# HazyResearch/flash-fft-conv

Measured on AMD Instinct MI355X. Metric: FFT-conv fwd+bwd seq/s, B=16 H=768 L=16384 fft=32768 bf16, higher is better.
Workload: dtype bf16; 1 GPU; FlashFFTConv(32768) B=16 H=768 L=16384 bf16, fwd+bwd incl. k->k_f and dk (BASELINE configs[1]); heads_per_rank=768, parallelism=head-shard x1 (no collective)

## Files before the change

flash-fft-conv_amd/csrc/ffc_body.h:

```cpp
#pragma once
#include <stdint.h>

#include "ffc_layout.h"
#include "ffc_plan.h"

#ifndef FFC_FN
#define FFC_FN inline __attribute__((always_inline))
#endif

namespace ffc {

struct ConvArgs {
  const void* u;
  const void* pregate;
  const void* postgate;
  void* y;
  const void* kf;
  const uint8_t* tab;
  PlanTabs t;
  int B, H, L;
  int npair;
  int nchunk, ppc;
  int conj_kf;
  int fast;
// ... 562 lines not shown
    else rows_load<NC>(a, h, pq, un, X);
  }
  template <int NC, bool PL>
  static FFC_FN void rows_store_sel(const ConvArgs& a, int h, int pq, Unit un, const RowRegsT<NC>& X) {
    if constexpr (PL) rows_store_pl<NC>(a, pq, un, X);
    else rows_store<NC>(a, h, pq, un, X);
  }
  template <int NC, bool PL>
  static FFC_FN void rows_in_sel(const ConvArgs& a, int h, int pq, Unit un) {
    RowRegsT<NC> X;
    rows_load_sel<NC, PL>(a, h, pq, un, X);
    rows_store_sel<NC, PL>(a, h, pq, un, X);
  }
  static constexpr bool HAS_DMA = GEO::OUTER && GEO::N1 == 32 && GEO::S1 == 1;
  static constexpr int DMA_ROW0 = GEO::N1 / 2;
  static FFC_FN void rows_dma(const ConvArgs& a, int h, int pq, Unit un) {
    if (a.stream) rows_dma_t<true>(a, h, pq, un);
    else rows_dma_t<false>(a, h, pq, un);
  }
  template <bool NT>
  static FFC_FN void rows_dma_t(const ConvArgs& a, int h, int pq, Unit un) {
    const i32 lane = B::opaque(B::lane());
#pragma unroll
    for (int pl = 0; pl < 2; pl++) {
      const int b = 2 * pq + pl;
      const uint16_t* base = (const uint16_t*)a.u + row_off(b < a.B ? b : a.B - 1, true, a.sbu, h, a.L);
#pragma unroll
      for (int r = 0; r < GEO::N1 / 2; r++) {
        i32 n = B::imin(lane * 2 + (r * GEO::Mi + un.wq * 128), a.L - 2);
        B::template g2lds32<NT>(base, n >> 1, un.eb + pl * GEO::PLANE + (DMA_ROW0 + r) * (GEO::Mi * 2) + un.wq * 256);
      }
    }
  }
  static FFC_FN void rows_dma_finish(const ConvArgs& a, int pq, Unit un) {
    B::vm_wait0();
    const i32 lane = B::opaque(B::lane());
#pragma unroll
    for (int pl = 0; pl < 2; pl++) {
      const bool ok = (2 * pq + pl) < a.B;
#pragma unroll
      for (int r = 0; r < GEO::N1 / 2; r++) {
        if (ok && (r + 1) * GEO::Mi <= a.L) continue;
        i32 n = lane * 2 + (r * GEO::Mi + un.wq * 128);
        B::lds_w32p(lane * 4 + (un.eb + pl * GEO::PLANE + (DMA_ROW0 + r) * (GEO::Mi * 2) + un.wq * 256), B::uconst(0),
                    B::pnot((n < a.L) && ok));
      }
    }
    B::lds_fence();
  }

  static FFC_FN U4 gload8_rows(const uint16_t* base, i32 b, int h, const ConvArgs& a, int64_t sb, i32 n, int fast, pred ok) {
    const int sbi = (int)sb;
    if (fast) {
      i32 o16 = b * (sbi >> 3) + (h * (a.L >> 3) + (n >> 3));
      return B::g_r128p(base, o16, ok && (n < a.L));
    }
    u32 w[4];
#pragma unroll
    for (int q = 0; q < 4; q++) {
      i32 e0 = b * sbi + (h * a.L + n + 2 * q);
      u32 lo = B::g_r16(base, e0, ok && ((n + 2 * q) < a.L));
      u32 hi = B::g_r16(base, e0 + 1, ok && ((n + (2 * q + 1)) < a.L));
      w[q] = lo | (hi << 16);
    }
    U4 v; v.x = w[0]; v.y = w[1]; v.z = w[2]; v.w = w[3];
    return v;
  }
  static FFC_FN void gstore8_rows(uint16_t* base, i32 b, int h, const ConvArgs& a, int64_t sb, i32 n, int fast, pred ok, U4 v) {
// ... 597 lines not shown
            i32 m = j * 4 + (s1 * 128 + w * 128 * GEO::S1 + 2 * tp + th);
            i32 k0 = hi * 4 + ((16 * half) % GEO::N1);
            F2 tr[4], ti[4];
            if constexpr (RP) chain8p(m * (k0 * ps.R + ps.k0), m * ps.R, -1.0f, s_fwd, tr, ti, GEO::N * ps.R - 1, 1.0f / (float)(GEO::N * ps.R));
            else chain8p(m * k0, m, -1.0f, s_fwd, tr, ti);
            apply8(re, im, half, tr, ti);
          }
        }
        if (th == 0) {
          re0 = re; im0 = im;
        } else {
#pragma unroll
          for (int r = 0; r < 16; r++) {
            if (!FWD && HALF && row_dead((r & 3) + 8 * (r >> 2))) continue;
            const u32 vr = B::template pack<DT>(re0[r], re[r]), vi = B::template pack<DT>(im0[r], im[r]);
            if (tp == 0) {
              p0r[r] = vr; p0i[r] = vi;
            } else {
              const int c = (r & 3) + 8 * (r >> 2);
              const int s1 = c / GEO::N1, rwc = c % GEO::N1;
              i32 off = colb[s1] + rwc * (GEO::Mi * 2);
              U2 wr, wi;
              wr.x = p0r[r]; wr.y = vr; wi.x = p0i[r]; wi.y = vi;
              B::lds_w64(off, wr);
              B::lds_w64(off + GEO::PLANE, wi);
            }
          }
        }
      }
    }
  }

  static constexpr bool HALF_C = GEO::N1 == 32 && GEO::N2 == 32 && GEO::N3 == 32;
  using A4 = typename B::A4;
  struct NoMid { FFC_FN void operator()() const {} };
  template <bool GS, class MID>
  static FFC_FN void outer_inv_half_cols(int hc, Unit un, const W4& Cr, const W4& Ci, const W4& Cn, const ConvArgs* a, int h, int pq, MID mid) {
    const i32 lane = B::opaque(B::lane());
    const i32 c = lane & 15, g = lane >> 4;
    const i32 m0 = c * 4 + (hc * 64 + un.wq * 128);
    const i32 colr = e_off<GEO, i32>((g >> 1) * 16 + (g & 1) * 4, m0) + un.eb;
    U2 rawr[8], rawi[8];
#pragma unroll
    for (int e = 0; e < 8; e++) {
      i32 off = colr + kslot_row(0, 0, e) * (GEO::Mi * 2);
      rawr[e] = B::lds_r64(off); rawi[e] = B::lds_r64(off + GEO::PLANE);
    }
    A4 re[4], im[4];
#pragma unroll
    for (int t = 0; t < 4; t++) {
      W4 dr, di;
#pragma unroll
      for (int d = 0; d < 4; d++) {
        const u32 ar = (t & 2) ? rawr[2 * d].y : rawr[2 * d].x, br = (t & 2) ? rawr[2 * d + 1].y : rawr[2 * d + 1].x;
        const u32 ai = (t & 2) ? rawi[2 * d].y : rawi[2 * d].x, bi = (t & 2) ? rawi[2 * d + 1].y : rawi[2 * d + 1].x;
        dr[d] = (t & 1) ? B::merge_hi(ar, br) : B::merge_lo(ar, br);
        di[d] = (t & 1) ? B::merge_hi(ai, bi) : B::merge_lo(ai, bi);
      }
      re[t] = B::a4_zero(); im[t] = B::a4_zero();
      B::template mfma16<DT>(re[t], Cr, dr);
      B::template mfma16<DT>(im[t], Ci, dr);
      B::template mfma16<DT>(re[t], Cn, di);
      B::template mfma16<DT>(im[t], Cr, di);
      if (t == 0) mid();
    }
    U2 wr[4], wi[4];
#pragma unroll
    for (int r = 0; r < 4; r++) {
      wr[r].x = B::template pack<DT>(re[0][r], re[1][r]); wr[r].y = B::template pack<DT>(re[2][r], re[3][r]);
      wi[r].x = B::template pack<DT>(im[0][r], im[1][r]); wi[r].y = B::template pack<DT>(im[2][r], im[3][r]);
    }
    if constexpr (!GS) {
      const i32 colw = e_off<GEO, i32>(g * 4, m0) + un.eb;
#pragma unroll
      for (int r = 0; r < 4; r++) {
        B::lds_w64(colw + r * (GEO::Mi * 2), wr[r]);
        B::lds_w64(colw + (r * (GEO::Mi * 2) + GEO::PLANE), wi[r]);
      }
    } else {
      const i32 n = g * (4 * GEO::Mi) + m0;
#pragma unroll
      for (int pl = 0; pl < 2; pl++) {
        const int b = 2 * pq + pl;
        const bool ok = b < a->B;
        uint16_t* base = (uint16_t*)a->y + row_off(b, ok, a->sby, h, a->L);
        if (a->stream) {
#pragma unroll
          for (int r = 0; r < 4; r++) B::g_w64_nt(base, (n + r * GEO::Mi) >> 2, pl ? wi[r] : wr[r], ((n + r * GEO::Mi) < a->L) && ok);
        } else {
#pragma unroll
          for (int r = 0; r < 4; r++) B::g_w64(base, (n + r * GEO::Mi) >> 2, pl ? wi[r] : wr[r], ((n + r * GEO::Mi) < a->L) && ok);
        }
      }
    }
  }
  template <bool GS>
  static FFC_FN void outer_inv_half(Unit un, const ConvArgs* a = nullptr, int h = 0, int pq = 0) { outer_inv_half<GS>(un, a, h, pq, NoMid()); }
  template <bool GS, class LAST>
  static FFC_FN void outer_inv_half(Unit un, const ConvArgs* a, int h, int pq, LAST last) {
    static_assert(HALF_C && GEO::S1 == 1 && GEO::NW == 8, "half-height phase C: fft 32768");
    static_assert(!GS || !B::HAS_ADD, "the direct store has no addend");
    const i32 lane = B::opaque(B::lane());
    const i32 toff = ((lane & 15) + ((lane >> 4) & 1) * 32) * 16 + (lane >> 5) * 3072 + GEO::L_F1;
    U4 v0 = B::lds_r128(toff), v1 = B::lds_r128(toff + 1024), v2 = B::lds_r128(toff + 2048);
    W4 Cr = B::w4(v0.x, v0.y, v0.z, v0.w);
    W4 Ci = B::w4(v2.x, v2.y, v2.z, v2.w);
    W4 Cn = B::w4(v1.x, v1.y, v1.z, v1.w);
    B::pin(Cr); B::pin(Ci); B::pin(Cn);
    if constexpr (B::LEAN_OUTER) {
#pragma unroll 1
      for (int hc = 0; hc < 2; hc++)
        outer_inv_half_cols<GS>(hc, un, Cr, Ci, Cn, a, h, pq, [&]() { if (hc == 1) last(); });
    } else {
      outer_inv_half_cols<GS>(0, un, Cr, Ci, Cn, a, h, pq, NoMid());
      outer_inv_half_cols<GS>(1, un, Cr, Ci, Cn, a, h, pq, last);
    }
  }

  template <bool FWD, bool HALF, bool RP = false, bool DIN = false, bool NOTW = false>
  static FFC_FN void outer_stage(int L, Unit un, float s_fwd = 1.0f, Pass ps = Pass(), int flags = 0) {
    if constexpr (DIN) { outer_stage_pair<FWD, HALF, RP, true, NOTW>(L, un, s_fwd, ps); return; }
    if constexpr (!FWD && HALF && !RP && HALF_C) {
      if (!(flags & 256)) { outer_inv_half<false>(un); return; }
    }
    if constexpr (B::LEAN_OUTER && !(FWD && HALF && GEO::N1 == 32)) outer_stage_tile<FWD, HALF, RP, NOTW>(L, un, s_fwd, ps);
    else if constexpr (!B::LEAN_OUTER && FFC_OUTER_QUAD != 0 && HALF) outer_stage_quad<FWD, HALF, RP, NOTW>(L, un, s_fwd, ps);
    else outer_stage_pair<FWD, HALF, RP, false, NOTW>(L, un, s_fwd, ps);
  }

  struct InnerRegs { Mat F2; CT16 tw; i32 roff[2][2]; i32 woff[4]; };
  template <bool TWR = true>
  static FFC_FN void load_inner(InnerRegs& R, Unit un) {
    lds_mat(R.F2, GEO::L_F2);
    if constexpr (TWR) lds_ct16(R.tw, GEO::L_TW);
    const i32 lane = B::lane();
    const i32 c = lane & 31, hi = lane >> 5;
    const i32 i16 = lane & 15, g16 = (lane >> 4) & 1;
    const i32 n3b = (g16 * 16) % GEO::N3;
#pragma unroll
    for (int ms = 0; ms < 2; ms++)
#pragma unroll
      for (int rho = 0; rho < 2; rho++) {
        i32 U = hi * 4 + (16 * ms + 8 * rho) + (i16 >> 2);
        i32 sU = U / GEO::N2, n2 = U % GEO::N2;
        i32 row = sU * GEO::SV + ((g16 * 16) / GEO::N3);
        R.roff[ms][rho] = e_off<GEO, i32>(row, n2 * GEO::N3 + n3b + (i16 & 3) * 4) + un.eb;
      }
#pragma unroll
// ... 684 lines not shown
        for (int i = 0; i < 4; i++) B::cmulp(tr[i], ti[i], c16, s16, tr[i], ti[i]);
        apply8(reA, imA, 1, tr, ti);
        apply8(reB, imB, 1, tr, ti);
      } else
#pragma unroll
      for (int half = 0; half < 2; half++) {
        const int sV = (16 * half) / GEO::N3;
        i32 k1 = sUl * GEO::SV + (sV + tau * GEO::G);
        i32 n30 = hi * 4 + ((16 * half) % GEO::N3);
        F2 tr[4], ti[4];
        chain8p(B::mul24(mlane + n30, k1), k1, 1.0f, a.s_inv, tr, ti);
        apply8(reA, imA, half, tr, ti);
        apply8(reB, imB, half, tr, ti);
      }
    }
    tile_store(tau, R, reA, imA);
    tile_store(tau, R, reB, imB, DB);
  }

  static FFC_FN void unit_barrier() {
    if constexpr (GEO::NW > 1) B::barrier();
    else B::lds_fence();
  }
  template <bool HALF, bool PROF = false, bool RP = false, bool SZ = false, bool SP = false, bool GS = false, bool PL = false>
  static FFC_FN void outer_jobs(const ConvArgs& a, int h, int p0, int p1, int u, Unit un, int wg_linear = 0) {
    static_assert(!GS || (HALF && !RP && !SP && HALF_C), "direct-store phase C: single-pass fft 32768, L <= N/2");
    static_assert(!PL || GS, "plain input rows: a form of the direct-store kernels");
    constexpr int NC = HALF ? NCH / 2 : NCH;
    constexpr bool PREFETCH = HALF && !RP;
    constexpr bool FOLDF = CAN_FOLD && !RP && !SP && !PROF && !B::LEAN_OUTER;
    constexpr bool CROSS = !SP && !RP && !PROF && !B::LEAN_OUTER && GEO::N3 == GEO::N2 && GEO::NW > 1 && GEO::UPW >= 2;
    const int npass = RP ? a.R : 1;
    const int iters = ((p1 - p0 + GEO::UPW - 1) / GEO::UPW) * npass;
    RowRegsT<NC> X;
    if constexpr (PREFETCH) { if (p0 + u < p1) rows_load_sel<NC, PL>(a, h, p0 + u, un, X); }
    unsigned long long acc[8] = {0, 0, 0, 0, 0, 0, 0, 0}, t0 = 0, t1 = 0;
#define FFC_TICK(k) if (PROF) { t1 = B::clock(); acc[k] += t1 - t0; t0 = t1; }
    const bool second = B::wave() >= 4;
#define FFC_PRIO(x) if constexpr (GEO::NW > 1) B::template setprio<x>();
#pragma unroll 1
    for (int it = 0; it < iters; it++) {
      const int p = p0 + (RP ? it / npass : it) * GEO::UPW + u;
      const Pass ps = RP ? make_pass(a, it % npass) : Pass();
      const int hk = RP ? h * ps.R + ps.k0 : h;
      const bool act = (PL && GEO::UPW == 1) || p < p1;
      if (PROF) t0 = B::clock();
      FFC_PRIO(1)
      if (act) {
        if constexpr (RP) {
          rows_in_rp<NC>(a, h, p, un, ps);
        } else {
          if constexpr (!PREFETCH) rows_load_sel<NC, PL>(a, h, p, un, X);
          rows_store_sel<NC, PL>(a, h, p, un, X);
        }
        B::lds_fence();
        FFC_TICK(0)
        FFC_PRIO(0)
        outer_stage<true, HALF, RP, false, FOLDF>(a.L, un, a.s_fwd, ps);
        FFC_TICK(1)
      }
      unit_barrier();
      FFC_TICK(2)
      if constexpr (CROSS) {
        const int ug = u >> 1, wl = (u & 1) * GEO::NW + un.wq;
        const int pA = p0 + it * GEO::UPW + 2 * ug;
        if (pA < p1) {
          Unit ua;
          ua.eb = 2 * ug * GEO::EBYTES; ua.wq = wl;
          InnerRegs R;
          load_inner(R, ua);
          uint8_t* zA = SZ ? z_slot(a.zsave, h, a.npair, pA) : nullptr;
          if (pA + 1 < p1) {
#pragma unroll 1
            for (int tt = 0; tt < 2; tt++) {
              if (tt == 0) { FFC_PRIO(3) } else if (second) { FFC_PRIO(2) } else { FFC_PRIO(1) }
              if constexpr (FOLDF) inner_tile2x_fold<SZ>(a, hk, wl * 2 + tt, R, ua, zA, zA + (int64_t)GEO::N * 4);
              else inner_tile2x<SZ>(a, hk, wl * 2 + tt, R, ua, zA, zA + (int64_t)GEO::N * 4);
            }
          } else {
            inner_tile2<false, SZ, FOLDF, HALF>(a, hk, wl * 2, R, ua, Pass(), zA);
          }
        }
      } else if (act) {
        InnerRegs R;
        load_inner(R, un);
        if constexpr (SP) {
          Mat Fs;
          lds_mat_sp(Fs);
#pragma unroll 1
          for (int tt = 0; tt < GEO::TPW; tt += 2) inner_tile2_sp(a, hk, un.wq * GEO::TPW + tt, R, Fs, un);
        } else if constexpr (GEO::N3 == GEO::N2) {
#pragma unroll 1
          for (int tt = 0; tt < GEO::TPW; tt += 2) {
            if (tt == 0) { FFC_PRIO(3) } else if (second) { FFC_PRIO(2) } else { FFC_PRIO(1) }
            inner_tile2<RP, SZ, FOLDF, HALF>(a, hk, un.wq * GEO::TPW + tt, R, un, ps,
                                SZ ? (RP ? z_slot_rp(a.zsave, h, a.npair, p, ps.R, ps.k0) : z_slot(a.zsave, h, a.npair, p)) : nullptr);
          }
        } else {
          KfRegs kf0;
          load_kf(a, h, un.wq * GEO::TPW, kf0);
#pragma unroll 1
          for (int tt = 0; tt < GEO::TPW; tt++) {
            KfRegs kfn;
            if (tt + 1 < GEO::TPW) load_kf(a, h, un.wq * GEO::TPW + tt + 1, kfn);
            inner_tile(a, un.wq * GEO::TPW + tt, R, un, kf0);
            kf0 = kfn;
          }
        }
      }
      FFC_TICK(3)
      unit_barrier();
      FFC_TICK(4)
      FFC_PRIO(3)
      if constexpr (PREFETCH) { if (it + 1 < iters && p + GEO::UPW < p1) rows_load_sel<NC, PL>(a, h, p + GEO::UPW, un, X); }
      if constexpr (GS) {
        if (act) {
          outer_inv_half<true>(un, &a, h, p);
          FFC_TICK(5)
        }
      } else if (act) {
        outer_stage<false, HALF, RP>(a.L, un, 1.0f, ps, a.flags);
        B::lds_fence();
        FFC_TICK(5)
        FFC_PRIO(2)
        if constexpr (SZ) {
          if (a.yraw) {
            ConvArgs ar = a;
            ar.y = a.yraw; ar.postgate = nullptr; ar.addend = nullptr; ar.sby = (int64_t)a.H * a.L;
            if constexpr (RP) rows_out_rp<NC, false>(ar, h, p, un, ps);
            else rows_out<NC, false>(ar, h, p, un);
          }
        }
        if constexpr (RP) rows_out_rp<NC>(a, h, p, un, ps);
        else rows_out<NC>(a, h, p, un);
        FFC_TICK(6)
      }
    }
#undef FFC_TICK
#undef FFC_PRIO
    if (PROF && a.prof) {
      const i32 lane = B::lane();
      unsigned long long* dst = a.prof + ((long long)wg_linear * GEO::WGW + B::wave()) * 8;
#pragma unroll
      for (int k = 0; k < 8; k++) B::g_w64(dst, lane * 0 + k, B::u2_from64(acc[k]), lane < 1);
    }
  }

  template <bool HALF = false, bool SZ = false, bool SP = false, bool GS = false, bool PL = false>
  static FFC_FN void conv(const ConvArgs& a, int h, int chunk) {
    setup_tables(a.tab, a.t);
    conv_job<HALF, false, SZ, SP, GS, PL>(a, h, chunk);
// ... 166 lines not shown
```

flash-fft-conv_amd/csrc/ffc_dev.h:

```cpp
#pragma once
#include <hip/hip_runtime.h>
#include <stdint.h>
#include <stdlib.h>
#include <string.h>

#include <string>
#include <type_traits>

#define FFC_FN __device__ __forceinline__
#include "../../include/flashfftconv_hip.h"
#include "ffc_body.h"
#include "ffc_modes.h"
#include "ffc_big.h"
#include "ffc_route.h"

namespace ffc {

typedef __bf16 bf16x8 __attribute__((ext_vector_type(8)));
typedef _Float16 f16x8 __attribute__((ext_vector_type(8)));
typedef __bf16 bf16x2 __attribute__((ext_vector_type(2)));
typedef _Float16 f16x2 __attribute__((ext_vector_type(2)));
typedef float f32x2 __attribute__((ext_vector_type(2)));
typedef float f32x16 __attribute__((ext_vector_type(16)));
typedef short s16x4 __attribute__((ext_vector_type(4)));
// ... 79 lines not shown
  static FFC_FN u32 as_u32(f32 a) { return __builtin_bit_cast(uint32_t, a); }

  static FFC_FN U2 lds_r64(i32 off) { uint2 v = *(const uint2*)(ffc_smem + off); return U2{v.x, v.y}; }
  static FFC_FN void lds_w64(i32 off, U2 v) { *(uint2*)(ffc_smem + off) = make_uint2(v.x, v.y); }
  static FFC_FN void lds_w32(i32 off, u32 v) { *(uint32_t*)(ffc_smem + off) = v; }
  static FFC_FN void lds_w128(i32 off, U4 v, pred p) {
    if (p) *(uint4*)(ffc_smem + off) = make_uint4(v.x, v.y, v.z, v.w);
  }
  static FFC_FN U4 lds_r128(i32 off) { uint4 v = *(const uint4*)(ffc_smem + off); return U4{v.x, v.y, v.z, v.w}; }
  static FFC_FN void lds_w16(i32 off, u32 v) { *(uint16_t*)(ffc_smem + off) = (uint16_t)v; }
  static FFC_FN u32 lds_r32(i32 off) { return *(const uint32_t*)(ffc_smem + off); }
  static FFC_FN u32 lds_r16(i32 off) { return *(const uint16_t*)(ffc_smem + off); }
  static FFC_FN U2 lds_r64_tr(i32 off) {
    s16x4 t = __builtin_amdgcn_ds_read_tr16_b64_v4i16((__attribute__((address_space(3))) s16x4*)(ffc_smem + off));
    uint2 v = __builtin_bit_cast(uint2, t);
    return U2{v.x, v.y};
  }
  static FFC_FN void lds_fence() { __builtin_amdgcn_fence(__ATOMIC_ACQ_REL, "wavefront"); }
  template <bool NT>
  static FFC_FN void g2lds32(const void* base, i32 dw, int lds_off) {
    const __attribute__((address_space(1))) void* g = (const __attribute__((address_space(1))) void*)((const uint32_t*)base + dw);
    __attribute__((address_space(3))) void* l = (__attribute__((address_space(3))) void*)(ffc_smem + lds_off);
    if constexpr (NT) __builtin_amdgcn_global_load_lds(g, l, 4, 0, 2);
    else __builtin_amdgcn_global_load_lds(g, l, 4, 0, 0);
  }
  template <bool NT>
  static FFC_FN void g2lds128(const void* base, i32 o16, int lds_off) {
    const __attribute__((address_space(1))) void* g = (const __attribute__((address_space(1))) void*)((const uint4*)base + o16);
    __attribute__((address_space(3))) void* l = (__attribute__((address_space(3))) void*)(ffc_smem + lds_off);
    if constexpr (NT) __builtin_amdgcn_global_load_lds(g, l, 16, 0, 2);
    else __builtin_amdgcn_global_load_lds(g, l, 16, 0, 0);
  }
  static FFC_FN void vm_wait0() { __builtin_amdgcn_s_waitcnt(0x0F70); }
  static FFC_FN void lds_wait0() { __builtin_amdgcn_s_waitcnt(0xC07F); __builtin_amdgcn_sched_barrier(0); }
  static FFC_FN void lds_w32p(i32 off, u32 v, pred p) { if (p) *(uint32_t*)(ffc_smem + off) = v; }
  static FFC_FN pred pnot(pred p) { return !p; }
  static FFC_FN u32 uconst(uint32_t c) { return c; }
  static FFC_FN i32 mul24(i32 a, i32 b) { return __mul24(a, b); }
  static FFC_FN unsigned long long clock() { return __builtin_amdgcn_s_memtime(); }
  template <int P> static FFC_FN void setprio() { __builtin_amdgcn_s_setprio(P); }
  static FFC_FN U2 u2_from64(unsigned long long v) { return U2{(u32)v, (u32)(v >> 32)}; }
  static FFC_FN void settle(f32& a, f32& b) { asm volatile("s_nop 4" : "+v"(a), "+v"(b)); }
  static FFC_FN f32 i2f(i32 a) { return (float)a; }
  static FFC_FN f32 cos_rev(f32 x) { return __builtin_amdgcn_cosf(x); }
  static FFC_FN f32 sin_rev(f32 x) { return __builtin_amdgcn_sinf(x); }
  static FFC_FN i32 opaque(i32 x) { asm volatile("" : "+v"(x)); return x; }
  static FFC_FN u32 sel(pred p, u32 a, u32 b) { return p ? a : b; }
  static FFC_FN u32 merge_lo(u32 a, u32 b) { return __builtin_amdgcn_perm(b, a, 0x05040100u); }
  static FFC_FN u32 merge_hi(u32 a, u32 b) { return __builtin_amdgcn_perm(b, a, 0x07060302u); }
  static FFC_FN i32 imin(i32 a, int b) { return a < b ? a : b; }
  static FFC_FN u32 g_r16(const void* base, i32 e, pred p) {
    uint16_t v = 0;
    if (p) v = ((const uint16_t*)base)[e];
    return v;
  }
  static FFC_FN void g_w16(void* base, i32 e, u32 v, pred p) {
    if (p) ((uint16_t*)base)[e] = (uint16_t)v;
  }
  static FFC_FN u32 g_r32(const void* base, i32 e, pred p) {
    uint32_t v = 0;
    if (p) v = ((const uint32_t*)base)[e];
    return v;
  }
  static FFC_FN void g_w32(void* base, i32 e, u32 v, pred p) {
    if (p) ((uint32_t*)base)[e] = v;
  }
  static FFC_FN U2 g_r64(const void* base, i32 o8, pred p) {
    uint2 v = make_uint2(0, 0);
    if (p) v = ((const uint2*)base)[o8];
    return U2{v.x, v.y};
  }
  static FFC_FN void g_w64(void* base, i32 o8, U2 v, pred p) {
    if (p) ((uint2*)base)[o8] = make_uint2(v.x, v.y);
  }
  static FFC_FN void g_w64_nt(void* base, i32 o8, U2 v, pred p) {
    if (p) { u32x2v t = {v.x, v.y}; __builtin_nontemporal_store(t, ((u32x2v*)base) + o8); }
  }
  static FFC_FN U4 g_r128(const void* base, i32 o16) {
    uint4 v = ((const uint4*)base)[o16];
    return U4{v.x, v.y, v.z, v.w};
  }
  static FFC_FN U4 g_r128_nt(const void* base, i32 o16) {
    u32x4v v = __builtin_nontemporal_load(((const u32x4v*)base) + o16);
    return U4{v.x, v.y, v.z, v.w};
  }
  static FFC_FN void g_w128_nt(void* base, i32 o16, U4 v, pred p) {
    if (p) { u32x4v t = {v.x, v.y, v.z, v.w}; __builtin_nontemporal_store(t, ((u32x4v*)base) + o16); }
  }
  static FFC_FN U4 g_r128p(const void* base, i32 o16, pred p) {
    uint4 v = make_uint4(0, 0, 0, 0);
    if (p) v = ((const uint4*)base)[o16];
    return U4{v.x, v.y, v.z, v.w};
  }
  static FFC_FN void g_w128(void* base, i32 o16, U4 v, pred p) {
    if (p) ((uint4*)base)[o16] = make_uint4(v.x, v.y, v.z, v.w);
  }
  template <int DT>
  static FFC_FN void mfma(A16& acc, const W4& a, const W4& b) {
    if (DT == DT_BF16)
      acc = __builtin_amdgcn_mfma_f32_32x32x16_bf16(__builtin_bit_cast(bf16x8, a), __builtin_bit_cast(bf16x8, b), acc, 0, 0, 0);
    else
      acc = __builtin_amdgcn_mfma_f32_32x32x16_f16(__builtin_bit_cast(f16x8, a), __builtin_bit_cast(f16x8, b), acc, 0, 0, 0);
  }
  template <int DT>
  static FFC_FN void mfma16(A4& acc, const W4& a, const W4& b) {
    if (DT == DT_BF16)
      acc = __builtin_amdgcn_mfma_f32_16x16x32_bf16(__builtin_bit_cast(bf16x8, a), __builtin_bit_cast(bf16x8, b), acc, 0, 0, 0);
    else
      acc = __builtin_amdgcn_mfma_f32_16x16x32_f16(__builtin_bit_cast(f16x8, a), __builtin_bit_cast(f16x8, b), acc, 0, 0, 0);
// ... 145 lines not shown
```

flash-fft-conv_amd/csrc/ffc_modes.h:

```cpp
#pragma once
#include "ffc_body.h"

namespace ffc {

struct KfArgs {
  const float* k;
  void* kf;
  const uint8_t* tab;
  PlanTabs t;
  int H, Lk;
  float scale;
  float s_fwd;
  float prescale;
  const void* xpair;
  int fast;
  int R;
};

struct DkfArgs {
  ConvArgs c;
  const void* dout;
  float* ws;
  int64_t sbd, sbdu, sbdpre, sbdpost;
  void* du;
// ... 852 lines not shown
    un.wq = wv % GEO::NW;
    const int u = wv / GEO::NW;
    un.eb = u * GEO::EBYTES;
    const int p0 = chunk * a.ppc;
    int p1 = p0 + a.ppc;
    if (p1 > a.npair) p1 = a.npair;
    ConvArgs av = a;
    ConvArgs ad = a;
    ad.u = d.dout; ad.pregate = a.postgate; ad.sbu = d.sbd; ad.sbg = a.sbp;
    ConvArgs ao = a;
    ao.y = d.du; ao.postgate = a.pregate; ao.sby = d.sbdu; ao.sbp = a.sbg;
    ConvArgs ap = a;
    ap.y = d.dpre; ap.postgate = a.u; ap.sby = d.sbdpre; ap.sbp = a.sbu;
    ConvArgs aq = a;
    aq.y = d.dpost; aq.postgate = d.dout; aq.sby = d.sbdpost; aq.sbp = d.sbd;
    const bool dpost_tf = !PL && d.dpost != nullptr && d.yraw == nullptr;
    if constexpr (!(RP && GEO::OUTER) && !PL) {
      if (d.dpost && d.yraw) { ad.aux_in = d.yraw; ad.aux_out = d.dpost; ad.sbai = (int64_t)a.H * a.L; ad.sbao = d.sbdpost; }
    }
    float* slab = RP ? d.ws + (((int64_t)chunk * a.H + h) * a.R + k0) * (GEO::NT * 2048)
                     : d.ws + ((int64_t)chunk * a.H + h) * (GEO::NT * 2048);
    InnerRegs R;
    if constexpr (GEO::OUTER) {
      const int iters = (p1 - p0 + GEO::UPW - 1) / GEO::UPW;
      uint8_t* zs = (uint8_t*)d.zscratch + ((int64_t)(wg_linear * GEO::UPW + u)) * (GEO::N * 4);
      WAcc W;
      w_acc_zero(W);
      const bool have_z = ZM < 0 ? d.zin != nullptr : ZM == 1;
      constexpr bool FOLDZ = BD::CAN_FOLD && GEO::N1 == 32 && ZM == 1 && !RP;
      constexpr bool DMA_OK = BD::HAS_DMA && HALF && !RP && ZM != 0;
      static_assert(!PL || ZM == 0 || DMA_OK, "plain rows on saved spectra: the rows come by LDS-DMA");
      const bool dma = DMA_OK && (PL || (have_z && a.fast && !ad.pregate && !ad.aux_in && !dpost_tf && !(a.flags & 8)));
      if constexpr (DMA_OK) { if (dma && p0 + u < p1) BD::rows_dma(ad, h, p0 + u, un); }
      const bool second = wv >= 4;
#define FFC_BPRIO(x) if constexpr (GEO::NW > 1) B::template setprio<x>();
#pragma unroll 1
      for (int it = 0; it < iters; it++) {
        const int p = p0 + it * GEO::UPW + u;
        const bool act = (PL && GEO::UPW == 1) || p < p1;
        FFC_BPRIO(1)
        const void* zp = !have_z ? (const void*)zs
                         : RP ? (const void*)BD::z_slot_rp(const_cast<void*>(d.zin), h, a.npair, act ? p : p0, a.R, k0)
                              : (const void*)BD::z_slot(const_cast<void*>(d.zin), h, a.npair, act ? p : p0);
        if (have_z) {
          if (dpost_tf) {
            BD::unit_barrier();
            if (act) {
              BD::template load_inner<false>(R, un);
#pragma unroll 1
              for (int tt = 0; tt < GEO::TPW; tt++) {
                const int tau = un.wq * GEO::TPW + tt;
                typename BD::KfRegs zv, kf;
                z_load(zp, tau, zv, BD::Z_STREAM);
                BD::load_kf(a, hk, tau, kf);
                A16 re, im;
                z_unpack(zv, re, im);
                kf_plain_mul(kf, re, im);
                BD::template tile_inv<false, RP>(a.s_inv, tau, R, un, re, im, 0, ps);
              }
            }
            BD::unit_barrier();
            if (act) {
              BD::template outer_stage<false, HALF, RP>(a.L, un, 1.0f, ps, a.flags);
              B::lds_fence();
              if constexpr (RP) BD::template rows_out_rp<NCX>(aq, h, p, un, ps);
              else BD::template rows_out<NCX>(aq, h, p, un);
            }
          }
          if (act) {
            bool done = false;
            if constexpr (DMA_OK) {
              if (dma) {
                BD::rows_dma_finish(ad, p, un);
                FFC_BPRIO(0)
                BD::template outer_stage<true, HALF, RP, true, FOLDZ>(a.L, un, a.s_fwd, ps);
                done = true;
              }
            }
            if (!done) {
              if constexpr (RP) BD::template rows_in_rp<NCX>(ad, h, p, un, ps);
              else BD::template rows_in_sel<NCX, PL>(ad, h, p, un);
              B::lds_fence();
              FFC_BPRIO(0)
              BD::template outer_stage<true, HALF, RP, false, FOLDZ>(a.L, un, a.s_fwd, ps);
            }
          }
        } else {
          if (act) {
            if constexpr (RP) BD::template rows_in_rp<NCX>(av, h, p, un, ps);
            else BD::template rows_in_sel<NCX, PL>(av, h, p, un);
            B::lds_fence();
            FFC_BPRIO(0)
            BD::template outer_stage<true, HALF, RP>(a.L, un, a.s_fwd, ps);
          }
          BD::unit_barrier();
          FFC_BPRIO(3)
          if (act) {
            BD::template load_inner<false>(R, un);
#pragma unroll 1
            for (int tt = 0; tt < GEO::TPW; tt++) {
              const int tau = un.wq * GEO::TPW + tt;
              A16 re, im;
              BD::template tile_fwd<false>(tau, R, un, re, im);
              z_store(zs, tau, re, im, (a.flags & 4) != 0);
              if (dpost_tf) {
                typename BD::KfRegs kf;
// ... 4 lines not shown
            }
          }
          BD::unit_barrier();
          FFC_BPRIO(1)
          if (dpost_tf) {
            if (act) {
              BD::template outer_stage<false, HALF, RP>(a.L, un, 1.0f, ps, a.flags);
              B::lds_fence();
              if constexpr (RP) BD::template rows_out_rp<NCX>(aq, h, p, un, ps);
              else BD::template rows_out<NCX>(aq, h, p, un);
            }
          }
          if (act) {
            if constexpr (RP) BD::template rows_in_rp<NCX>(ad, h, p, un, ps);
            else BD::template rows_in_sel<NCX, PL>(ad, h, p, un);
            B::lds_fence();
            FFC_BPRIO(0)
            BD::template outer_stage<true, HALF, RP>(a.L, un, a.s_fwd, ps);
          }
        }
        BD::unit_barrier();
        FFC_BPRIO(3)
        if (act) {
          BD::template load_inner<false>(R, un);
          bwd_tiles<true, RP, ZM == 1>(a, hk, un, R, zp, slab, it == 0, W, ps, have_z && BD::Z_STREAM, second);
        } else if (it == 0) {
#pragma unroll 1
          for (int tt = GEO::TPW; tt < GEO::TPW; tt++) w_zero(slab, un.wq * GEO::TPW + tt);
        }
        BD::unit_barrier();
        FFC_BPRIO(3)
        if constexpr (GS) {
          if (act) {
            BD::template outer_inv_half<true>(un, &ao, h, p, [&]() {
              if constexpr (DMA_OK) {
                if (dma && p + GEO::UPW < p1) { B::lds_wait0(); BD::rows_dma(ad, h, p + GEO::UPW, un); }
              }
            });
          }
        } else if (act) {
          BD::template outer_stage<false, HALF, RP>(a.L, un, 1.0f, ps, a.flags);
          B::lds_fence();
          if constexpr (DMA_OK) { if (dma && p + GEO::UPW < p1) BD::rows_dma(ad, h, p + GEO::UPW, un); }
          FFC_BPRIO(2)
          if constexpr (RP) {
            BD::template rows_out_rp<NCX>(ao, h, p, un, ps);
            if (d.dpre) BD::template rows_out_rp<NCX>(ap, h, p, un, ps);
          } else {
            BD::template rows_out<NCX>(ao, h, p, un);
            if (d.dpre) BD::template rows_out<NCX>(ap, h, p, un);
          }
        }
      }
#undef FFC_BPRIO
      if constexpr (!RP && GEO::NW > 1) {
        if (d.dk_out || d.dk_pair) {
          using MB = Modes<B, GEO, DT_BF16>;
          if constexpr (DT != DT_BF16) {
            B::barrier();
            if constexpr (PL) MB::BD::setup_tables(d.tab_bf, d.t_bf, wv);
            else MB::BD::setup_tables(d.tab_bf, d.t_bf);
          }
          if constexpr (GEO::UPW == 1) MB::dk_tail(d, h, un.wq);
          else MB::dk_tail_multi(d, h, u, un.wq);
          return;
        }
      }
      if constexpr (RP && GEO::NW > 1 && GEO::UPW == 1 && DT == DT_BF16) {
        if (d.dk_out) { dk_tail_rp(d, h, un.wq, ps); return; }
      }
      w_acc_finish(slab, u, un, W);
// ... 370 lines not shown
```

flash-fft-conv_amd/csrc/ffc_sim.cpp:

```cpp
#include <math.h>
#include <pthread.h>
#include <stdint.h>
#include <stdlib.h>
#include <string.h>

#include <atomic>
#include <thread>
#include <vector>

#define FFC_FN inline __attribute__((always_inline))
#include "ffc_body.h"
#include "ffc_modes.h"
#include "ffc_big.h"
#include "ffc_route.h"

namespace ffc {

template <class T>
struct Vec {
  T v[64];
  Vec() {}
  Vec(T s) { for (int i = 0; i < 64; i++) v[i] = s; }
};
#define VOP(op)                                                                           \
// ... 138 lines not shown
    return r;
  }
  static u32 lds_r16(const i32& off) {
    u32 r;
    for (int i = 0; i < 64; i++) { chk(off.v[i], 2); uint16_t h; memcpy(&h, L() + off.v[i], 2); r.v[i] = h; }
    return r;
  }
  static U2 lds_r64_tr(const i32& off) {
    U2 r;
    for (int g = 0; g < 4; g++) {
      uint16_t M[16][4];
      for (int i = 0; i < 16; i++) { chk(off.v[g * 16 + i], 8); memcpy(M[i], L() + off.v[g * 16 + i], 8); }
      for (int i = 0; i < 16; i++) {
        uint16_t e[4];
        for (int j = 0; j < 4; j++) e[j] = M[4 * j + (i >> 2)][i & 3];
        r.x.v[g * 16 + i] = e[0] | ((uint32_t)e[1] << 16);
        r.y.v[g * 16 + i] = e[2] | ((uint32_t)e[3] << 16);
      }
    }
    return r;
  }
  static void lds_fence() {}
  template <bool NT>
  static void g2lds32(const void* base, const i32& dw, int lds_off) {
    g_dma_count++;
    for (int i = 0; i < 64; i++) { chk(lds_off + 4 * i, 4); memcpy(L() + lds_off + 4 * i, (const uint32_t*)base + dw.v[i], 4); }
  }
  template <bool NT>
  static void g2lds128(const void* base, const i32& o16, int lds_off) {
    g_dma_count++;
    for (int i = 0; i < 64; i++) { chk(lds_off + 16 * i, 16); memcpy(L() + lds_off + 16 * i, (const uint8_t*)base + 16 * (int64_t)o16.v[i], 16); }
  }
  static void vm_wait0() {}
  static void lds_wait0() {}
  static void lds_w32p(const i32& off, const u32& v, const pred& p) {
    for (int i = 0; i < 64; i++) if (p.v[i]) { chk(off.v[i], 4); memcpy(L() + off.v[i], &v.v[i], 4); }
  }
  static pred pnot(const pred& p) { pred r; for (int i = 0; i < 64; i++) r.v[i] = !p.v[i]; return r; }
  static i32 mul24(const i32& a, const i32& b) { return a * b; }
  static unsigned long long clock() { return 0; }
  template <int P> static void setprio() {}
  static U2 u2_from64(unsigned long long v) { U2 r; r.x = u32((uint32_t)v); r.y = u32((uint32_t)(v >> 32)); return r; }
  static void settle(f32&, f32&) {}
  static f32 i2f(const i32& a) { f32 r; for (int i = 0; i < 64; i++) r.v[i] = (float)a.v[i]; return r; }
  static f32 cos_rev(const f32& a) { f32 r; for (int i = 0; i < 64; i++) r.v[i] = (float)cos(6.283185307179586 * (double)a.v[i]); return r; }
  static f32 sin_rev(const f32& a) { f32 r; for (int i = 0; i < 64; i++) r.v[i] = (float)sin(6.283185307179586 * (double)a.v[i]); return r; }
  static i32 opaque(const i32& x) { return x; }
  static u32 uconst(uint32_t c) { return u32(c); }
  static i32 imin(const i32& a, int b) { i32 r; for (int i = 0; i < 64; i++) r.v[i] = a.v[i] < b ? a.v[i] : b; return r; }
  static u32 merge_lo(const u32& a, const u32& b) { u32 r; for (int i = 0; i < 64; i++) r.v[i] = (a.v[i] & 0xffffu) | (b.v[i] << 16); return r; }
  static u32 merge_hi(const u32& a, const u32& b) { u32 r; for (int i = 0; i < 64; i++) r.v[i] = (a.v[i] >> 16) | (b.v[i] & 0xffff0000u); return r; }
  static u32 sel(const pred& p, const u32& a, const u32& b) { u32 r; for (int i = 0; i < 64; i++) r.v[i] = p.v[i] ? a.v[i] : b.v[i]; return r; }
  static u32 g_r16(const void* base, const i32& e, const pred& p) {
    u32 r;
    for (int i = 0; i < 64; i++) { uint16_t h = 0; if (p.v[i]) memcpy(&h, (const uint8_t*)base + (int64_t)e.v[i] * 2, 2); r.v[i] = h; }
    return r;
  }
  static void g_w16(void* base, const i32& e, const u32& v, const pred& p) {
    for (int i = 0; i < 64; i++) if (p.v[i]) { uint16_t h = (uint16_t)v.v[i]; memcpy((uint8_t*)base + (int64_t)e.v[i] * 2, &h, 2); }
  }
  static u32 g_r32(const void* base, const i32& e, const pred& p) {
    u32 r;
    for (int i = 0; i < 64; i++) { uint32_t h = 0; if (p.v[i]) memcpy(&h, (const uint8_t*)base + (int64_t)e.v[i] * 4, 4); r.v[i] = h; }
    return r;
  }
  static void g_w32(void* base, const i32& e, const u32& v, const pred& p) {
    for (int i = 0; i < 64; i++) if (p.v[i]) memcpy((uint8_t*)base + (int64_t)e.v[i] * 4, &v.v[i], 4);
  }
  static U2 g_r64(const void* base, const i32& o8, const pred& p) {
    U2 r;
    for (int i = 0; i < 64; i++) {
      if (p.v[i]) { const uint8_t* q = (const uint8_t*)base + (int64_t)o8.v[i] * 8; memcpy(&r.x.v[i], q, 4); memcpy(&r.y.v[i], q + 4, 4); }
      else { r.x.v[i] = 0; r.y.v[i] = 0; }
    }
    return r;
  }
  static void g_w64(void* base, const i32& o8, const U2& v, const pred& p) {
    for (int i = 0; i < 64; i++)
      if (p.v[i]) { uint8_t* q = (uint8_t*)base + (int64_t)o8.v[i] * 8; memcpy(q, &v.x.v[i], 4); memcpy(q + 4, &v.y.v[i], 4); }
  }
  static void g_w64_nt(void* base, const i32& o8, const U2& v, const pred& p) { g_w64(base, o8, v, p); }
  static U4 g_r128(const void* base, const i32& o16) {
    U4 r;
    for (int i = 0; i < 64; i++) {
      const uint8_t* q = (const uint8_t*)base + (int64_t)o16.v[i] * 16;
      memcpy(&r.x.v[i], q, 4); memcpy(&r.y.v[i], q + 4, 4); memcpy(&r.z.v[i], q + 8, 4); memcpy(&r.w.v[i], q + 12, 4);
    }
    return r;
  }
  static U4 g_r128_nt(const void* base, const i32& o16) { return g_r128(base, o16); }
  static U4 g_r128p(const void* base, const i32& o16, const pred& p) {
    U4 r;
    for (int i = 0; i < 64; i++) {
      if (p.v[i]) {
        const uint8_t* q = (const uint8_t*)base + (int64_t)o16.v[i] * 16;
        memcpy(&r.x.v[i], q, 4); memcpy(&r.y.v[i], q + 4, 4); memcpy(&r.z.v[i], q + 8, 4); memcpy(&r.w.v[i], q + 12, 4);
      } else { r.x.v[i] = r.y.v[i] = r.z.v[i] = r.w.v[i] = 0; }
    }
    return r;
  }
// ... 643 lines not shown
```

Before: 11.54 million seq/s.

## Rotate pair loop: finish next rows' DMA after output stores, using buffer stores

In the plain-rows paths, the pair loop is rotated so the next pair's row load (LDS-DMA finish or prefetched row store) happens right after the current pair's output stores rather than at the top of the next iteration. The DMA wait now uses a partial vmcnt that leaves the just-issued output stores outstanding. The output stores switch to raw buffer stores whose bounds come from the resource descriptor, which removes per-lane predication. The aim is to overlap global stores with the next input's arrival. The vmcnt arithmetic depends on counting the stores exactly, so a miscount would read rows before they land.

```diff
diff --git a/flash-fft-conv_amd/csrc/ffc_body.h b/flash-fft-conv_amd/csrc/ffc_body.h
--- a/flash-fft-conv_amd/csrc/ffc_body.h
+++ b/flash-fft-conv_amd/csrc/ffc_body.h
@@ -618,8 +618,12 @@
       }
     }
   }
+  static constexpr int DMA_COPIES = 2 * (GEO::N1 / 2);
+  template <int BEHIND = 0>
   static FFC_FN void rows_dma_finish(const ConvArgs& a, int pq, Unit un) {
-    B::vm_wait0();
+    static_assert(BEHIND >= 0 && BEHIND + DMA_COPIES <= 63, "vmcnt is a 6-bit counter: the copies and what follows them must fit");
+    if constexpr (BEHIND == 0) B::vm_wait0();
+    else B::template vm_wait<BEHIND>();
     const i32 lane = B::opaque(B::lane());
 #pragma unroll
     for (int pl = 0; pl < 2; pl++) {
@@ -1283,9 +1287,11 @@
   }
 
   static constexpr bool HALF_C = GEO::N1 == 32 && GEO::N2 == 32 && GEO::N3 == 32;
+  static constexpr int HALF_C_ROWS = 4;
+  static constexpr int HALF_C_STORES = 2 * HALF_C_ROWS;
   using A4 = typename B::A4;
   struct NoMid { FFC_FN void operator()() const {} };
-  template <bool GS, class MID>
+  template <bool GS, bool UN, class MID>
   static FFC_FN void outer_inv_half_cols(int hc, Unit un, const W4& Cr, const W4& Ci, const W4& Cn, const ConvArgs* a, int h, int pq, MID mid) {
     const i32 lane = B::opaque(B::lane());
     const i32 c = lane & 15, g = lane >> 4;
@@ -1315,9 +1321,9 @@
       B::template mfma16<DT>(im[t], Cr, di);
       if (t == 0) mid();
     }
-    U2 wr[4], wi[4];
-#pragma unroll
-    for (int r = 0; r < 4; r++) {
+    U2 wr[HALF_C_ROWS], wi[HALF_C_ROWS];
+#pragma unroll
+    for (int r = 0; r < HALF_C_ROWS; r++) {
       wr[r].x = B::template pack<DT>(re[0][r], re[1][r]); wr[r].y = B::template pack<DT>(re[2][r], re[3][r]);
       wi[r].x = B::template pack<DT>(im[0][r], im[1][r]); wi[r].y = B::template pack<DT>(im[2][r], im[3][r]);
     }
@@ -1335,20 +1341,27 @@
         const int b = 2 * pq + pl;
         const bool ok = b < a->B;
         uint16_t* base = (uint16_t*)a->y + row_off(b, ok, a->sby, h, a->L);
+        if constexpr (UN) {
+          const int nb = ok ? a->L * 2 : 0;
+#pragma unroll
+          for (int r = 0; r < HALF_C_ROWS; r++) B::template row_w64<true>(base, nb, (n + r * GEO::Mi) * 2, pl ? wi[r] : wr[r]);
+          continue;
+        }
         if (a->stream) {
 #pragma unroll
-          for (int r = 0; r < 4; r++) B::g_w64_nt(base, (n + r * GEO::Mi) >> 2, pl ? wi[r] : wr[r], ((n + r * GEO::Mi) < a->L) && ok);
+          for (int r = 0; r < HALF_C_ROWS; r++) B::g_w64_nt(base, (n + r * GEO::Mi) >> 2, pl ? wi[r] : wr[r], ((n + r * GEO::Mi) < a->L) && ok);
         } else {
 #pragma unroll
-          for (int r = 0; r < 4; r++) B::g_w64(base, (n + r * GEO::Mi) >> 2, pl ? wi[r] : wr[r], ((n + r * GEO::Mi) < a->L) && ok);
-        }
-      }
-    }
-  }
-  template <bool GS>
-  static FFC_FN void outer_inv_half(Unit un, const ConvArgs* a = nullptr, int h = 0, int pq = 0) { outer_inv_half<GS>(un, a, h, pq, NoMid()); }
-  template <bool GS, class LAST>
+          for (int r = 0; r < HALF_C_ROWS; r++) B::g_w64(base, (n + r * GEO::Mi) >> 2, pl ? wi[r] : wr[r], ((n + r * GEO::Mi) < a->L) && ok);
+        }
+      }
+    }
+  }
+  template <bool GS, bool UN = false>
+  static FFC_FN void outer_inv_half(Unit un, const ConvArgs* a = nullptr, int h = 0, int pq = 0) { outer_inv_half<GS, UN>(un, a, h, pq, NoMid()); }
+  template <bool GS, bool UN, class LAST>
   static FFC_FN void outer_inv_half(Unit un, const ConvArgs* a, int h, int pq, LAST last) {
+    static_assert(!UN || GS, "unconditional stores: a form of the direct store");
     static_assert(HALF_C && GEO::S1 == 1 && GEO::NW == 8, "half-height phase C: fft 32768");
     static_assert(!GS || !B::HAS_ADD, "the direct store has no addend");
     const i32 lane = B::opaque(B::lane());
@@ -1361,10 +1374,10 @@
     if constexpr (B::LEAN_OUTER) {
 #pragma unroll 1
       for (int hc = 0; hc < 2; hc++)
-        outer_inv_half_cols<GS>(hc, un, Cr, Ci, Cn, a, h, pq, [&]() { if (hc == 1) last(); });
+        outer_inv_half_cols<GS, UN>(hc, un, Cr, Ci, Cn, a, h, pq, [&]() { if (hc == 1) last(); });
     } else {
-      outer_inv_half_cols<GS>(0, un, Cr, Ci, Cn, a, h, pq, NoMid());
-      outer_inv_half_cols<GS>(1, un, Cr, Ci, Cn, a, h, pq, last);
+      outer_inv_half_cols<GS, UN>(0, un, Cr, Ci, Cn, a, h, pq, NoMid());
+      outer_inv_half_cols<GS, UN>(1, un, Cr, Ci, Cn, a, h, pq, last);
     }
   }
 
@@ -2115,12 +2128,22 @@
     constexpr bool CROSS = !SP && !RP && !PROF && !B::LEAN_OUTER && GEO::N3 == GEO::N2 && GEO::NW > 1 && GEO::UPW >= 2;
     const int npass = RP ? a.R : 1;
     const int iters = ((p1 - p0 + GEO::UPW - 1) / GEO::UPW) * npass;
+    constexpr bool ROT = PL && PREFETCH;
+    static_assert(!ROT || GEO::UPW == 1, "rotated pair loop: one unit owns the workgroup, every iteration has its pair");
     RowRegsT<NC> X;
     if constexpr (PREFETCH) { if (p0 + u < p1) rows_load_sel<NC, PL>(a, h, p0 + u, un, X); }
     unsigned long long acc[8] = {0, 0, 0, 0, 0, 0, 0, 0}, t0 = 0, t1 = 0;
 #define FFC_TICK(k) if (PROF) { t1 = B::clock(); acc[k] += t1 - t0; t0 = t1; }
     const bool second = B::wave() >= 4;
 #define FFC_PRIO(x) if constexpr (GEO::NW > 1) B::template setprio<x>();
+    if constexpr (ROT) {
+      if (p0 + u < p1) {
+        if (PROF) t0 = B::clock();
+        FFC_PRIO(1)
+        rows_store_pl<NC>(a, p0 + u, un, X);
+        FFC_TICK(0)
+      }
+    }
 #pragma unroll 1
     for (int it = 0; it < iters; it++) {
       const int p = p0 + (RP ? it / npass : it) * GEO::UPW + u;
@@ -2128,11 +2151,11 @@
       const int hk = RP ? h * ps.R + ps.k0 : h;
       const bool act = (PL && GEO::UPW == 1) || p < p1;
       if (PROF) t0 = B::clock();
-      FFC_PRIO(1)
+      if constexpr (!ROT) { FFC_PRIO(1) }
       if (act) {
         if constexpr (RP) {
           rows_in_rp<NC>(a, h, p, un, ps);
-        } else {
+        } else if constexpr (!ROT) {
           if constexpr (!PREFETCH) rows_load_sel<NC, PL>(a, h, p, un, X);
           rows_store_sel<NC, PL>(a, h, p, un, X);
         }
@@ -2198,8 +2221,15 @@
       if constexpr (PREFETCH) { if (it + 1 < iters && p + GEO::UPW < p1) rows_load_sel<NC, PL>(a, h, p + GEO::UPW, un, X); }
       if constexpr (GS) {
         if (act) {
-          outer_inv_half<true>(un, &a, h, p);
+          outer_inv_half<true, ROT>(un, &a, h, p);
           FFC_TICK(5)
+        }
+        if constexpr (ROT) {
+          if (it + 1 < iters && p + GEO::UPW < p1) {
+            FFC_PRIO(1)
+            rows_store_pl<NC>(a, p + GEO::UPW, un, X);
+            FFC_TICK(0)
+          }
         }
       } else if (act) {
         outer_stage<false, HALF, RP>(a.L, un, 1.0f, ps, a.flags);
diff --git a/flash-fft-conv_amd/csrc/ffc_dev.h b/flash-fft-conv_amd/csrc/ffc_dev.h
--- a/flash-fft-conv_amd/csrc/ffc_dev.h
+++ b/flash-fft-conv_amd/csrc/ffc_dev.h
@@ -135,6 +135,10 @@
     else __builtin_amdgcn_global_load_lds(g, l, 16, 0, 0);
   }
   static FFC_FN void vm_wait0() { __builtin_amdgcn_s_waitcnt(0x0F70); }
+  template <int N> static FFC_FN void vm_wait() {
+    static_assert(N >= 0 && N <= 63, "vmcnt is a 6-bit counter");
+    __builtin_amdgcn_s_waitcnt(0x0F70 | (N & 15) | ((N >> 4) << 14));
+  }
   static FFC_FN void lds_wait0() { __builtin_amdgcn_s_waitcnt(0xC07F); __builtin_amdgcn_sched_barrier(0); }
   static FFC_FN void lds_w32p(i32 off, u32 v, pred p) { if (p) *(uint32_t*)(ffc_smem + off) = v; }
   static FFC_FN pred pnot(pred p) { return !p; }
@@ -178,6 +182,12 @@
   }
   static FFC_FN void g_w64_nt(void* base, i32 o8, U2 v, pred p) {
     if (p) { u32x2v t = {v.x, v.y}; __builtin_nontemporal_store(t, ((u32x2v*)base) + o8); }
+  }
+  template <bool NT>
+  static FFC_FN void row_w64(void* row, int nbytes, i32 off, U2 v) {
+    __amdgpu_buffer_rsrc_t r = __builtin_amdgcn_make_buffer_rsrc(row, 0, nbytes, 0x00020000);
+    u32x2v t = {v.x, v.y};
+    __builtin_amdgcn_raw_buffer_store_b64(t, r, off, 0, NT ? 2 : 0);
   }
   static FFC_FN U4 g_r128(const void* base, i32 o16) {
     uint4 v = ((const uint4*)base)[o16];
diff --git a/flash-fft-conv_amd/csrc/ffc_modes.h b/flash-fft-conv_amd/csrc/ffc_modes.h
--- a/flash-fft-conv_amd/csrc/ffc_modes.h
+++ b/flash-fft-conv_amd/csrc/ffc_modes.h
@@ -908,13 +908,21 @@
       static_assert(!PL || ZM == 0 || DMA_OK, "plain rows on saved spectra: the rows come by LDS-DMA");
       const bool dma = DMA_OK && (PL || (have_z && a.fast && !ad.pregate && !ad.aux_in && !dpost_tf && !(a.flags & 8)));
       if constexpr (DMA_OK) { if (dma && p0 + u < p1) BD::rows_dma(ad, h, p0 + u, un); }
+      constexpr bool ROT = PL && ZM == 1;
+      static_assert(!ROT || (DMA_OK && GEO::UPW == 1), "rotated pair loop: rows by LDS-DMA, one unit owns the workgroup");
       const bool second = wv >= 4;
 #define FFC_BPRIO(x) if constexpr (GEO::NW > 1) B::template setprio<x>();
+      if constexpr (ROT) {
+        if (p0 + u < p1) {
+          FFC_BPRIO(1)
+          BD::rows_dma_finish(ad, p0 + u, un);
+        }
+      }
 #pragma unroll 1
       for (int it = 0; it < iters; it++) {
         const int p = p0 + it * GEO::UPW + u;
         const bool act = (PL && GEO::UPW == 1) || p < p1;
-        FFC_BPRIO(1)
+        if constexpr (!ROT) { FFC_BPRIO(1) }
         const void* zp = !have_z ? (const void*)zs
                          : RP ? (const void*)BD::z_slot_rp(const_cast<void*>(d.zin), h, a.npair, act ? p : p0, a.R, k0)
                               : (const void*)BD::z_slot(const_cast<void*>(d.zin), h, a.npair, act ? p : p0);
@@ -947,7 +955,7 @@
             bool done = false;
             if constexpr (DMA_OK) {
               if (dma) {
-                BD::rows_dma_finish(ad, p, un);
+                if constexpr (!ROT) BD::rows_dma_finish(ad, p, un);
                 FFC_BPRIO(0)
                 BD::template outer_stage<true, HALF, RP, true, FOLDZ>(a.L, un, a.s_fwd, ps);
                 done = true;
@@ -1018,11 +1026,17 @@
         FFC_BPRIO(3)
         if constexpr (GS) {
           if (act) {
-            BD::template outer_inv_half<true>(un, &ao, h, p, [&]() {
+            BD::template outer_inv_half<true, ROT>(un, &ao, h, p, [&]() {
               if constexpr (DMA_OK) {
                 if (dma && p + GEO::UPW < p1) { B::lds_wait0(); BD::rows_dma(ad, h, p + GEO::UPW, un); }
               }
             });
+          }
+          if constexpr (ROT) {
+            if (p + GEO::UPW < p1) {
+              FFC_BPRIO(1)
+              BD::template rows_dma_finish<BD::HALF_C_STORES>(ad, p + GEO::UPW, un);
+            }
           }
         } else if (act) {
           BD::template outer_stage<false, HALF, RP>(a.L, un, 1.0f, ps, a.flags);
diff --git a/flash-fft-conv_amd/csrc/ffc_sim.cpp b/flash-fft-conv_amd/csrc/ffc_sim.cpp
--- a/flash-fft-conv_amd/csrc/ffc_sim.cpp
+++ b/flash-fft-conv_amd/csrc/ffc_sim.cpp
@@ -194,6 +194,7 @@
     for (int i = 0; i < 64; i++) { chk(lds_off + 16 * i, 16); memcpy(L() + lds_off + 16 * i, (const uint8_t*)base + 16 * (int64_t)o16.v[i], 16); }
   }
   static void vm_wait0() {}
+  template <int N> static void vm_wait() {}
   static void lds_wait0() {}
   static void lds_w32p(const i32& off, const u32& v, const pred& p) {
     for (int i = 0; i < 64; i++) if (p.v[i]) { chk(off.v[i], 4); memcpy(L() + off.v[i], &v.v[i], 4); }
@@ -228,6 +229,11 @@
   }
   static void g_w32(void* base, const i32& e, const u32& v, const pred& p) {
     for (int i = 0; i < 64; i++) if (p.v[i]) memcpy((uint8_t*)base + (int64_t)e.v[i] * 4, &v.v[i], 4);
+  }
+  template <bool NT>
+  static void row_w64(void* row, int nbytes, const i32& off, const U2& v) {
+    for (int i = 0; i < 64; i++)
+      if ((uint32_t)off.v[i] < (uint32_t)nbytes) { uint8_t* q = (uint8_t*)row + off.v[i]; memcpy(q, &v.x.v[i], 4); memcpy(q + 4, &v.y.v[i], 4); }
   }
   static U2 g_r64(const void* base, const i32& o8, const pred& p) {
     U2 r;
```

Result: faster. 11.69 million seq/s, median of 6 (+1.3%).
